# anihcsam/OpenGaussian

Measured on AMD Instinct MI355X. Metric: fwd+bwd Mpix/s at 1080p, 1M Gaussians (RGB+6-D ins_feat); k-means it/s, higher is better.
Workload: dtype f32; 1 GPU; S1M-1080p RGB(SH3)+depth+alpha (all grads) + 6-ch ins_feat (grad to ins_feat) fwd+bwd, ONE fused 9-channel pass; gaussians=1000000, width=1920, height=1080, views_cycled=8, parallelism=single

## Files before the change

include/ogs_raster.h:

```cpp
#ifndef OGS_RASTER_H
#define OGS_RASTER_H

#include <stddef.h>
#include <stdint.h>

#ifdef __cplusplus
extern "C" {
#endif

#define OGS_OK 0
#define OGS_ERR_INVALID_ARG (-1)
#define OGS_ERR_HIP (-2)
#define OGS_ERR_UNSUPPORTED (-3)
#define OGS_ERR_SCRATCH_TOO_SMALL (-4)
#define OGS_ERR_DEVICE (-5)

#define OGS_TILE 16
#define OGS_MAX_CHANNELS 12

typedef struct OgsRasterFwdArgs {
    int32_t P;
    int32_t W, H;
    int32_t C;
    int32_t sh_degree;
// ... 73 lines not shown
} OgsRasterBwdArgs;

int ogs_version(void);
const char* ogs_last_error(void);

int ogs_check_async_status(void);

size_t ogs_raster_geom_bytes(int32_t P, int32_t C);
size_t ogs_raster_geom_tmp_bytes(int32_t P);
size_t ogs_raster_image_bytes(int32_t W, int32_t H);
size_t ogs_raster_image_bytes_grouped(int32_t W, int32_t H, int32_t num_groups);
size_t ogs_raster_binning_tmp_bytes(int64_t num_rendered, int32_t W, int32_t H);
size_t ogs_raster_backward_tmp_bytes(int32_t P);
size_t ogs_raster_sorted_bytes(int64_t num_rendered, int32_t C);
size_t ogs_raster_quad_list_bytes(int64_t num_rendered);

int ogs_raster_forward_geometry(const OgsRasterFwdArgs* args, void* stream, int64_t* num_rendered_host);

int ogs_raster_forward_render(const OgsRasterFwdArgs* args, int64_t num_rendered, void* stream);

int ogs_raster_read_num_rendered_async(const OgsRasterFwdArgs* args, void* stream, uint32_t* host_pinned);
int ogs_raster_forward_render_deferred(const OgsRasterFwdArgs* args, int64_t capacity, void* stream);

int ogs_raster_read_num_emitted(const OgsRasterFwdArgs* args, void* stream, uint32_t* host);

size_t ogs_raster_tiny_max_points(void);
int ogs_raster_forward_tiny(const OgsRasterFwdArgs* args, void* stream);

size_t ogs_raster_tile_sort_capacity(int32_t level);

int ogs_raster_tile_count_debug(int64_t D, int64_t tiles, int32_t force_blocks, int32_t reverse);
size_t ogs_raster_tile_count_trip(void);

int ogs_raster_forward_reblend(const OgsRasterFwdArgs* args, void* stream);

int ogs_raster_compact_kept(int32_t W, int32_t H, int32_t C, const void* image_buffer, const void* sorted_rec,
                            const void* quad_list, void* new_image_buffer, void* new_sorted_rec, void* new_quad_list,
                            void* stream);

typedef struct OgsGroupStatsArgs {
    const int32_t* labels;
    int32_t num_labels;
    float alpha_threshold;
    float* max_alpha;
    int64_t* count;
    float* feat_sum;
    void* stats_tmp;
} OgsGroupStatsArgs;

size_t ogs_raster_stats_image_bytes(int32_t W, int32_t H, int32_t num_groups);
size_t ogs_raster_stats_tmp_bytes(int32_t num_groups, int32_t num_labels, int32_t C);
int ogs_raster_forward_group_stats(const OgsRasterFwdArgs* args, const OgsGroupStatsArgs* stats, int64_t num_rendered,
                                   void* stream);

int ogs_raster_backward(const OgsRasterBwdArgs* args, void* stream);

int ogs_mark_visible(int32_t P, const float* means3D, const float* viewmatrix, const float* projmatrix,
                     uint8_t* present, void* stream);

int ogs_sh_grad_from_views(int32_t P, int32_t V, int32_t sh_degree, int32_t sh_coeffs, const float* means3D,
                           const float* campos, const float* dL_drgb, float* dL_dsh, void* stream);

int ogs_raster_export_binning(const OgsRasterFwdArgs* args, int64_t num_rendered, uint64_t* keys_out,
                              uint32_t* ranges_out, uint32_t* n_contrib_out, void* stream);

int ogs_prof_enable(int on);
// ... 17 lines not shown
```

opengaussian_amd/_lib.py:

```python
from __future__ import annotations

import ctypes as C
import os

_HERE = os.path.dirname(os.path.abspath(__file__))
LIB_PATH = os.environ.get("OGS_LIB_PATH") or os.path.join(_HERE, "lib", "libogs_hip.so")

_f32p = C.POINTER(C.c_float)
_vp = C.c_void_p


class OgsRasterFwdArgs(C.Structure):
    _fields_ = [
        ("P", C.c_int32), ("W", C.c_int32), ("H", C.c_int32), ("C", C.c_int32),
        ("sh_degree", C.c_int32), ("sh_coeffs", C.c_int32),
        ("tanfovx", C.c_float), ("tanfovy", C.c_float), ("scale_modifier", C.c_float),
        ("prefiltered", C.c_int32), ("debug", C.c_int32),
        ("bg", _vp), ("means3D", _vp), ("colors_precomp", _vp), ("shs", _vp), ("opacities", _vp),
        ("scales", _vp), ("rotations", _vp), ("cov3D_precomp", _vp),
        ("viewmatrix", _vp), ("projmatrix", _vp), ("campos", _vp),
        ("out_color", _vp), ("out_depth", _vp), ("out_alpha", _vp), ("radii", _vp),
        ("geom_buffer", _vp), ("geom_tmp", _vp), ("image_buffer", _vp), ("point_list", _vp),
        ("binning_tmp", _vp), ("sorted_rec", _vp), ("quad_list", _vp), ("group_ids", _vp), ("num_groups", C.c_int32),
        ("full_binning", C.c_int32),
# ... 59 lines not shown

class OgsRawModel(C.Structure):
    _fields_ = [("features_dc", _vp), ("features_rest", _vp), ("scaling", _vp), ("rotation", _vp), ("opacity", _vp)]


class OgsRawModelGrads(C.Structure):
    _fields_ = [("features_dc", _vp), ("features_rest", _vp), ("scaling", _vp), ("rotation", _vp), ("opacity", _vp)]


SIGNATURES = {
    "ogs_version": (C.c_int, []),
    "ogs_last_error": (C.c_char_p, []),
    "ogs_raster_geom_bytes": (C.c_size_t, [C.c_int32, C.c_int32]),
    "ogs_raster_geom_tmp_bytes": (C.c_size_t, [C.c_int32]),
    "ogs_raster_image_bytes": (C.c_size_t, [C.c_int32, C.c_int32]),
    "ogs_raster_image_bytes_grouped": (C.c_size_t, [C.c_int32, C.c_int32, C.c_int32]),
    "ogs_raster_binning_tmp_bytes": (C.c_size_t, [C.c_int64, C.c_int32, C.c_int32]),
    "ogs_raster_backward_tmp_bytes": (C.c_size_t, [C.c_int32]),
    "ogs_raster_sorted_bytes": (C.c_size_t, [C.c_int64, C.c_int32]),
    "ogs_raster_quad_list_bytes": (C.c_size_t, [C.c_int64]),
    "ogs_raster_forward_geometry": (C.c_int, [C.POINTER(OgsRasterFwdArgs), _vp, C.POINTER(C.c_int64)]),
    "ogs_raster_forward_render": (C.c_int, [C.POINTER(OgsRasterFwdArgs), C.c_int64, _vp]),
    "ogs_raster_read_num_rendered_async": (C.c_int, [C.POINTER(OgsRasterFwdArgs), _vp, _vp]),
    "ogs_raster_forward_render_deferred": (C.c_int, [C.POINTER(OgsRasterFwdArgs), C.c_int64, _vp]),
    "ogs_raster_read_num_emitted": (C.c_int, [C.POINTER(OgsRasterFwdArgs), _vp, C.POINTER(C.c_uint32)]),
    "ogs_raster_stats_image_bytes": (C.c_size_t, [C.c_int32, C.c_int32, C.c_int32]),
    "ogs_raster_stats_tmp_bytes": (C.c_size_t, [C.c_int32, C.c_int32, C.c_int32]),
    "ogs_raster_forward_group_stats": (C.c_int, [C.POINTER(OgsRasterFwdArgs), C.POINTER(OgsGroupStatsArgs), C.c_int64, _vp]),
    "ogs_raster_backward": (C.c_int, [C.POINTER(OgsRasterBwdArgs), _vp]),
    "ogs_raster_tiny_max_points": (C.c_size_t, []),
    "ogs_raster_tile_sort_capacity": (C.c_size_t, [C.c_int32]),
    "ogs_raster_tile_count_debug": (C.c_int, [C.c_int64, C.c_int64, C.c_int32, C.c_int32]),
    "ogs_raster_tile_count_trip": (C.c_size_t, []),
    "ogs_raster_forward_tiny": (C.c_int, [C.POINTER(OgsRasterFwdArgs), _vp]),
    "ogs_raster_forward_reblend": (C.c_int, [C.POINTER(OgsRasterFwdArgs), _vp]),
    "ogs_raster_compact_kept": (C.c_int, [C.c_int32, C.c_int32, C.c_int32, _vp, _vp, _vp, _vp, _vp, _vp, _vp]),
    "ogs_mark_visible": (C.c_int, [C.c_int32, _vp, _vp, _vp, _vp, _vp]),
    "ogs_sh_grad_from_views": (C.c_int, [C.c_int32, C.c_int32, C.c_int32, C.c_int32, _vp, _vp, _vp, _vp, _vp]),
    "ogs_raster_export_binning": (C.c_int, [C.POINTER(OgsRasterFwdArgs), C.c_int64, _vp, _vp, _vp, _vp]),
    "ogs_selftest_wave_fold16": (C.c_int, [_vp, _vp, _vp]),
    "ogs_selftest_mfma_rank1": (C.c_int, [_vp, _vp, _vp, C.c_int32, _vp, _vp, _vp]),
    "ogs_selftest_tile_order": (C.c_int, [_vp, C.c_int64, _vp, _vp]),
    "ogs_selftest_radix_tmp_bytes": (C.c_size_t, [C.c_int64]),
    "ogs_selftest_radix_sort": (C.c_int, [_vp, _vp, _vp, _vp, C.c_int64, C.c_int32, C.c_int32, C.c_int32, _vp, _vp, _vp, _vp]),
    "ogs_raster_forward_geometry_raw": (C.c_int, [C.POINTER(OgsRasterFwdArgs), C.POINTER(OgsRawModel), _vp,
                                                  C.POINTER(C.c_int64)]),
    "ogs_raster_forward_tiny_raw": (C.c_int, [C.POINTER(OgsRasterFwdArgs), C.POINTER(OgsRawModel), _vp]),
    "ogs_raster_backward_raw": (C.c_int, [C.POINTER(OgsRasterBwdArgs), C.POINTER(OgsRawModel), C.POINTER(OgsRawModelGrads), _vp]),
    "ogs_model_activate": (C.c_int, [C.c_int32, C.c_int32, C.POINTER(OgsRawModel), _vp, _vp, _vp, _vp, _vp]),
    "ogs_check_async_status": (C.c_int, []),
    "ogs_prof_enable": (C.c_int, [C.c_int]),
    "ogs_prof_filter": (C.c_int, [C.c_char_p]),
    "ogs_prof_collect": (C.c_int, [C.c_char_p, C.c_size_t]),
    "ogs_kmeans_tmp_bytes": (C.c_size_t, [C.c_int64, C.c_int32, C.c_int32]),
    "ogs_kmeans_lloyd": (C.c_int, [_vp, C.c_int64, C.c_int32, _vp, C.c_int32, C.c_int32, C.c_int32, C.c_int32,
                                   _vp, C.c_int64, _vp, _vp]),
    "ogs_kmeans_assign": (C.c_int, [_vp, C.c_int64, C.c_int32, _vp, C.c_int32, _vp, C.c_int64, _vp]),
    "ogs_mask_feature_sums": (C.c_int, [_vp, _vp, _vp, C.c_int32, C.c_int32, C.c_int64, C.c_int32, _vp, _vp]),
    "ogs_mask_feature_sqdev": (C.c_int, [_vp, _vp, _vp, _vp, C.c_int32, C.c_int32, C.c_int64, _vp, _vp]),
    "ogs_mask_feature_sums_backward": (C.c_int, [_vp, _vp, _vp, _vp, _vp, C.c_int32, C.c_int32, C.c_int64, _vp, _vp, _vp]),
    "ogs_mask_cohesion": (C.c_int, [_vp, _vp, _vp, C.c_int32, C.c_int32, C.c_int64, _vp, _vp]),
    "ogs_mask_cohesion_backward": (C.c_int, [_vp, _vp, _vp, _vp, C.c_int32, C.c_int32, C.c_int64, _vp, _vp, _vp]),
    "ogs_label_feature_sums": (C.c_int, [_vp, _vp, _vp, C.c_int32, C.c_int32, C.c_int64, C.c_int32, _vp, _vp]),
    "ogs_label_feature_sqdev": (C.c_int, [_vp, _vp, _vp, _vp, C.c_int32, C.c_int32, C.c_int64, _vp, _vp]),
    "ogs_label_feature_sums_backward": (C.c_int, [_vp, _vp, _vp, _vp, _vp, C.c_int32, C.c_int32, C.c_int64, _vp, _vp, _vp]),
    "ogs_label_cohesion": (C.c_int, [_vp, _vp, _vp, C.c_int32, C.c_int32, C.c_int64, _vp, _vp]),
# ... 144 lines not shown
```

opengaussian_amd/csrc/binning.hip:

```cpp
#include <stdlib.h>
#include <string.h>

#include "ogs_common.h"

namespace ogs {

namespace {

constexpr size_t kSweepHeaderWords = 4 * 256 + 4 + 60;
constexpr int kScanItems = 8;
constexpr int kScanTile = kBlock * kScanItems;

__device__ __forceinline__ uint32_t wave_inclusive_scan(uint32_t v) {
#pragma unroll
    for (int d = 1; d < kWave; d <<= 1) {
        uint32_t t = __shfl_up(v, d, kWave);
        if (lane_id() >= d) v += t;
    }
    return v;
}

__device__ __forceinline__ uint32_t block_exclusive_scan(uint32_t v, uint32_t& total, uint32_t* wave_sums ) {
    const int wave = threadIdx.x >> 6;
    const uint32_t inc = wave_inclusive_scan(v);
    if (lane_id() == kWave - 1) wave_sums[wave] = inc;
    __syncthreads();
    uint32_t base = 0, tot = 0;
#pragma unroll
    for (int w = 0; w < kBlock / kWave; ++w) {
        const uint32_t s = wave_sums[w];
        if (w < wave) base += s;
        tot += s;
    }
    total = tot;
// ... 393 lines not shown
    const int64_t D = n_dev ? min((int64_t)*n_dev, D_cap) : D_cap;
    const int64_t i0 = ((int64_t)blockIdx.x * kBlock + threadIdx.x) * kRangeItems;
    if (i0 >= D) return;
    uint32_t k[kRangeItems];
    if (i0 + kRangeItems <= D) {
        const uint4 v = *reinterpret_cast<const uint4*>(tile_keys + i0);
        k[0] = v.x; k[1] = v.y; k[2] = v.z; k[3] = v.w;
    } else {
#pragma unroll
        for (int j = 0; j < kRangeItems; ++j) k[j] = i0 + j < D ? tile_keys[i0 + j] : 0u;
    }
    uint32_t prev = i0 > 0 ? tile_keys[i0 - 1] : 0u;
#pragma unroll
    for (int j = 0; j < kRangeItems; ++j) {
        const int64_t i = i0 + j;
        if (i < D) {
            const uint32_t cur = k[j];
            if (i == 0) {
                ranges[cur].x = 0;
            } else if (prev != cur) {
                ranges[prev].y = (uint32_t)i;
                ranges[cur].x = (uint32_t)i;
            }
            if (i == D - 1) ranges[cur].y = (uint32_t)D;
            prev = cur;
        }
    }
}

constexpr int kCountBlock = 1024;
constexpr int kCountItems = 4;
constexpr int kCountTrip = kCountBlock * kCountItems;
constexpr int kCountScanCols = 64, kCountScanGroups = 16;

__device__ __forceinline__ void tile_count_chunk(const uint32_t* __restrict__ n_dev, int64_t n_cap, int nchunks, int64_t& begin,
                                                 int64_t& end) {
    const int64_t n = n_dev ? min((int64_t)*n_dev, n_cap) : n_cap;
    const int64_t per = (n + nchunks - 1) / nchunks;
    const int64_t chunk = (per + kCountTrip - 1) / kCountTrip * kCountTrip;
    begin = min(n, (int64_t)blockIdx.x * chunk);
    end = min(n, begin + chunk);
}

__global__ __launch_bounds__(kCountBlock) void tile_count_kernel(const uint32_t* __restrict__ keys, int64_t n_cap,
                                                                 const uint32_t* __restrict__ n_dev, int tiles,
                                                                 uint32_t* __restrict__ table ) {
    extern __shared__ uint32_t count_lds[];
    int64_t begin, end;
    tile_count_chunk(n_dev, n_cap, (int)gridDim.x, begin, end);
    for (int t = threadIdx.x; t < tiles; t += kCountBlock) count_lds[t] = 0u;
    __syncthreads();
    for (int64_t i0 = begin + (int64_t)threadIdx.x * kCountItems; i0 < end; i0 += kCountTrip) {
        uint32_t k[kCountItems];
        if (i0 + kCountItems <= end) {
            const uint4 v = *reinterpret_cast<const uint4*>(keys + i0);
            k[0] = v.x; k[1] = v.y; k[2] = v.z; k[3] = v.w;
        } else {
#pragma unroll
            for (int j = 0; j < kCountItems; ++j) k[j] = i0 + j < end ? keys[i0 + j] : kDropKey;
        }
#pragma unroll
        for (int j = 0; j < kCountItems; ++j)
            if (k[j] < (uint32_t)tiles) atomicAdd(&count_lds[k[j]], 1u);
    }
    __syncthreads();
    uint32_t* row = table + (size_t)blockIdx.x * tiles;
    for (int t = threadIdx.x; t < tiles; t += kCountBlock) row[t] = count_lds[t];
}

__global__ __launch_bounds__(kCountScanCols * kCountScanGroups) void tile_count_scan_kernel(uint32_t* __restrict__ table, int nrows,
                                                                                            int tiles) {
    __shared__ uint32_t part[kCountScanGroups][kCountScanCols];
    const int c = threadIdx.x & (kCountScanCols - 1), g = threadIdx.x / kCountScanCols;
    const int t = blockIdx.x * kCountScanCols + c;
    const int per = (nrows + kCountScanGroups - 1) / kCountScanGroups;
    const int r0 = min(nrows, g * per), r1 = min(nrows, r0 + per);
    uint32_t sum = 0;
    if (t < tiles) {
#pragma unroll 8
        for (int r = r0; r < r1; ++r) sum += table[(size_t)r * tiles + t];
    }
    part[g][c] = sum;
    __syncthreads();
    uint32_t run = 0, total = 0;
#pragma unroll
    for (int j = 0; j < kCountScanGroups; ++j) {
        const uint32_t v = part[j][c];
        if (j < g) run += v;
        total += v;
    }
    if (t >= tiles) return;
    if (g == 0) table[(size_t)nrows * tiles + t] = total;
#pragma unroll 8
    for (int r = r0; r < r1; ++r) {
        uint32_t* p = table + (size_t)r * tiles + t;
        const uint32_t v = *p;
        *p = run;
        run += v;
    }
}

__global__ __launch_bounds__(kCountBlock) void tile_place_kernel(const uint32_t* __restrict__ keys, const uint32_t* __restrict__ vals,
                                                                 int64_t n_cap, const uint32_t* __restrict__ n_dev, int tiles,
                                                                 const uint32_t* __restrict__ table, uint2* __restrict__ ranges,
                                                                 uint32_t* __restrict__ kept, uint32_t* __restrict__ out,
                                                                 uint32_t out_cap, bool reverse) {
    extern __shared__ uint32_t count_lds[];
    __shared__ uint32_t wave_sums[kCountBlock / kWave];
    int64_t begin, end;
    tile_count_chunk(n_dev, n_cap, (int)gridDim.x, begin, end);
    if (begin >= end && blockIdx.x != 0) return;
    const uint32_t* totals = table + (size_t)gridDim.x * tiles;
    const uint32_t* row = table + (size_t)blockIdx.x * tiles;
    for (int t = threadIdx.x; t < tiles; t += kCountBlock) count_lds[t] = totals[t];
    __syncthreads();
    const int per = ((tiles + kCountBlock - 1) / kCountBlock) | 1;
    const int t0 = min(tiles, (int)threadIdx.x * per), t1 = min(tiles, t0 + per);
    uint32_t sum = 0;
    for (int t = t0; t < t1; ++t) sum += count_lds[t];
    const uint32_t inc = wave_inclusive_scan(sum);
    if (lane_id() == kWave - 1) wave_sums[threadIdx.x >> 6] = inc;
    __syncthreads();
    uint32_t run = inc - sum, total = 0;
#pragma unroll
    for (int w = 0; w < kCountBlock / kWave; ++w) {
        const uint32_t v = wave_sums[w];
        if (w < (int)(threadIdx.x >> 6)) run += v;
        total += v;
    }
    for (int t = t0; t < t1; ++t) {
        const uint32_t cnt = count_lds[t];
        count_lds[t] = run;
        run += cnt;
    }
    __syncthreads();
    if (blockIdx.x == 0) {
        for (int t = threadIdx.x; t < tiles; t += kCountBlock) {
            const uint32_t cnt = totals[t], start = count_lds[t];
            ranges[t] = cnt ? make_uint2(start, start + cnt) : make_uint2(0u, 0u);
        }
        if (threadIdx.x == 0) *kept = total;
    }
    for (int t = threadIdx.x; t < tiles; t += kCountBlock) count_lds[t] += row[t];
    __syncthreads();
    for (int64_t j0 = (int64_t)threadIdx.x * kCountItems; j0 < end - begin; j0 += kCountTrip) {
        uint32_t k[kCountItems], v[kCountItems];
        if (!reverse && begin + j0 + kCountItems <= end) {
            const uint4 kk = *reinterpret_cast<const uint4*>(keys + begin + j0);
            const uint4 vv = *reinterpret_cast<const uint4*>(vals + begin + j0);
            k[0] = kk.x; k[1] = kk.y; k[2] = kk.z; k[3] = kk.w;
            v[0] = vv.x; v[1] = vv.y; v[2] = vv.z; v[3] = vv.w;
        } else {
#pragma unroll
            for (int j = 0; j < kCountItems; ++j) {
                const int64_t i = reverse ? end - 1 - (j0 + j) : begin + j0 + j;
                const bool in = j0 + j < end - begin;
                k[j] = in ? keys[i] : kDropKey;
                v[j] = in ? vals[i] : 0u;
            }
        }
#pragma unroll
        for (int j = 0; j < kCountItems; ++j) {
            if (k[j] < (uint32_t)tiles) {
                const uint32_t pos = atomicAdd(&count_lds[k[j]], 1u);
                if (pos < out_cap) out[pos] = v[j];
            }
        }
    }
}

constexpr int kTileSortWaves = kBlock / kWave;
struct TileSortLds {
    uint32_t hist[kTileSortWaves][256];
    uint32_t dig_start[256];
    uint32_t base[256];
    uint32_t scan_sums[4];
    uint32_t red[2];
    uint2 range[kTileSortWaves];
    uint32_t kv[2 * kTileSortCap];
};
typedef __attribute__((address_space(3))) volatile uint32_t LdsWord;
typedef __attribute__((address_space(3))) unsigned long long LdsMask;
__device__ __forceinline__ LdsWord* lds_words(uint32_t* p) { return (LdsWord*)p; }
__device__ __forceinline__ LdsMask* wave_masks(TileSortLds& sm, int wave) { return (LdsMask*)(sm.kv + wave * 2 * kWaveSortCap); }

__device__ __forceinline__ void wave_rank_clear(LdsWord* hist, LdsMask* masks) {
    const int lane = threadIdx.x & (kWave - 1);
#pragma unroll
    for (int j = 0; j < 4; ++j) {
        hist[lane + j * kWave] = 0u;
        __hip_atomic_store(&masks[lane + j * kWave], 0ull, __ATOMIC_SEQ_CST, __HIP_MEMORY_SCOPE_WAVEFRONT);
    }
    __builtin_amdgcn_wave_barrier();
}

__device__ __forceinline__ void wave_rank(LdsWord* hist, LdsMask* masks, const uint32_t (&key)[kTileSortItems],
                                          uint32_t (&rank)[kTileSortItems], int ipl, int first, int m, int shift,
                                          uint32_t mask) {
    const int lane = threadIdx.x & (kWave - 1);
    const unsigned long long me = 1ull << lane;
// ... 558 lines not shown
        OGS_LAUNCH(radix_scatter_kernel<8>, dim3(nb), dim3(kBlock), 0, stream, keys_in, vals_in, keys_out, vals_out, n, n_dev,
                   shift, bits, (const uint32_t*)hist, (const uint32_t*)row_total, nb, drop, kept_out);
    }
    OGS_LAUNCH_CHECK(debug, stream);
    return OGS_OK;
}

int launch_tile_ranges(const uint32_t* tile_keys_sorted, int64_t D, uint2* ranges, int64_t tiles, hipStream_t s,
                       int debug, const uint32_t* n_dev, bool already_zeroed) {
    if (!already_zeroed) OGS_HIP_CHECK(hipMemsetAsync(ranges, 0, (size_t)tiles * sizeof(uint2), s));
    if (D <= 0) return OGS_OK;
    const int grid = (int)((D + (int64_t)kBlock * kRangeItems - 1) / ((int64_t)kBlock * kRangeItems));
    OGS_LAUNCH(tile_ranges_kernel, dim3(grid), dim3(kBlock), 0, s, tile_keys_sorted, D, n_dev, ranges);
    OGS_LAUNCH_CHECK(debug, s);
    return OGS_OK;
}

static int g_tile_count_force = 0;
static bool g_tile_place_reverse = false;
void tile_count_debug(int force_blocks, int reverse) {
    if (force_blocks >= 0) g_tile_count_force = force_blocks;
    if (reverse >= 0) g_tile_place_reverse = reverse != 0;
}
int tile_count_trip() { return kCountTrip; }

int tile_count_blocks(int64_t D, int64_t tiles) {
    if (tiles < 1 || tiles > kTileCountMaxTiles || D < 2 * tiles) return 0;
    const int64_t trips = (D + kCountTrip - 1) / kCountTrip;
    int64_t B = g_tile_count_force > 0 ? g_tile_count_force : (trips < kTileCountBlocks ? trips : kTileCountBlocks);
    if (B > D / tiles - 1) B = D / tiles - 1;
    return (int)B;
}

int launch_tile_count_binning(const uint32_t* keys, const uint32_t* vals, int64_t D, const uint32_t* n_dev, int B, int64_t tiles,
                              uint32_t* table, uint2* ranges, uint32_t* kept, uint32_t* point_list, hipStream_t s, int debug) {
    if (B < 1 || tiles < 1 || tiles > kTileCountMaxTiles || ((int64_t)B + 1) * tiles > D) {
        set_error("tile_count_binning: B=%d tiles=%lld D=%lld", B, (long long)tiles, (long long)D); return OGS_ERR_INVALID_ARG;
    }
    const size_t lds = (size_t)tiles * sizeof(uint32_t);
    OGS_LAUNCH(tile_count_kernel, dim3(B), dim3(kCountBlock), lds, s, keys, D, n_dev, (int)tiles, table);
    OGS_LAUNCH_CHECK(debug, s);
    const int cols = (int)((tiles + kCountScanCols - 1) / kCountScanCols);
    OGS_LAUNCH(tile_count_scan_kernel, dim3(cols), dim3(kCountScanCols * kCountScanGroups), 0, s, table, B, (int)tiles);
    OGS_LAUNCH_CHECK(debug, s);
    OGS_LAUNCH(tile_place_kernel, dim3(B), dim3(kCountBlock), lds, s, keys, vals, D, n_dev, (int)tiles, (const uint32_t*)table,
               ranges, kept, point_list, (uint32_t)D, g_tile_place_reverse);
    OGS_LAUNCH_CHECK(debug, s);
    return OGS_OK;
}

int launch_tile_depth_sort(const uint2* ranges, int64_t tiles, const uint32_t* tile_order, uint32_t* point_list,
                           const uint32_t* depth_keys, uint32_t* scratch, hipStream_t s, int debug) {
    if (tiles <= 0) return OGS_OK;
    if (tiles >= (1ll << 31)) { set_error("tile_depth_sort: %lld tiles", (long long)tiles); return OGS_ERR_UNSUPPORTED; }
    const unsigned grid = (unsigned)((tiles + kTileSortWaves - 1) / kTileSortWaves);
    OGS_LAUNCH(tile_depth_sort_kernel, dim3(grid), dim3(kBlock), 0, s, ranges, (int)tiles, tile_order, point_list, depth_keys,
               scratch);
    OGS_LAUNCH_CHECK(debug, s);
    return OGS_OK;
}

int launch_export_keys(const uint2* ranges, int tiles, const uint32_t* point_list, const float4* rec, int recv4,
                       uint64_t* keys_out, hipStream_t s) {
    OGS_LAUNCH(export_keys_kernel, dim3(tiles), dim3(kBlock), 0, s, ranges, point_list, rec, recv4, keys_out);
    OGS_LAUNCH_CHECK(0, s);
    return OGS_OK;
}

}
```

opengaussian_amd/csrc/capi.hip:

```cpp
#include <stdarg.h>
#include <stdlib.h>
#include <string.h>

#include <map>
#include <mutex>
#include <string>
#include <vector>

#include "ogs_common.h"

namespace ogs {

static thread_local char g_err[512] = "";

void set_error(const char* fmt, ...) {
    va_list ap;
    va_start(ap, fmt);
    vsnprintf(g_err, sizeof(g_err), fmt, ap);
    va_end(ap);
}

namespace {
struct ProfRec { const char* name; hipEvent_t start, stop; };
int g_prof_mode = 0;
// ... 424 lines not shown
        set_error("forward_reblend: NULL required pointer (colors_precomp, bg, out_*, image_buffer, sorted_rec, quad_list)");
        return OGS_ERR_INVALID_ARG;
    }
    const int rc = check_async_status("forward_reblend (entry)");
    if (rc != OGS_OK) return rc;
    const ImageState is = ImageState::carve(a->image_buffer, a->W, a->H, 1);
    return launch_reblend(*a, is, static_cast<hipStream_t>(stream_));
}

int ogs_raster_compact_kept(int32_t W, int32_t H, int32_t C, const void* image_buffer, const void* sorted_rec, const void* quad_list,
                            void* new_image_buffer, void* new_sorted_rec, void* new_quad_list, void* stream_) {
    if (W <= 0 || H <= 0) { set_error("compact_kept: bad sizes W=%d H=%d", W, H); return OGS_ERR_INVALID_ARG; }
    if (!image_buffer || !sorted_rec || !quad_list || !new_image_buffer || !new_sorted_rec || !new_quad_list) {
        set_error("compact_kept: NULL pointer"); return OGS_ERR_INVALID_ARG;
    }
    const ImageState is_old = ImageState::carve(const_cast<void*>(image_buffer), W, H, 1);
    const ImageState is_new = ImageState::carve(new_image_buffer, W, H, 1);
    return launch_compact_kept(W, H, C, is_old, is_new, sorted_rec, quad_list, new_sorted_rec, new_quad_list,
                               static_cast<hipStream_t>(stream_));
}

size_t ogs_raster_tiny_max_points(void) { return (size_t)kTinyMaxP; }

size_t ogs_raster_tile_sort_capacity(int32_t level) {
    return level == 0 ? (size_t)kWaveSortCap : level == 1 ? (size_t)kTileSortCap : 0;
}

int ogs_raster_tile_count_debug(int64_t D, int64_t tiles, int32_t force_blocks, int32_t reverse) {
    tile_count_debug(force_blocks, reverse);
    return tile_count_blocks(D, tiles);
}
size_t ogs_raster_tile_count_trip(void) { return (size_t)tile_count_trip(); }

static int forward_tiny_impl(const OgsRasterFwdArgs* a_in, void* stream_, bool raw, const float* raw_rest) {
    int rc = validate_fwd(a_in);
    if (rc != OGS_OK) return rc;
    OgsRasterFwdArgs a_raw;
    const OgsRasterFwdArgs* a = a_in;
    if (raw) { a_raw = *a_in; a_raw.cov3D_precomp = raw_rest; a = &a_raw; }
    if (a->P <= 0 || a->P > kTinyMaxP) { set_error("forward_tiny: P=%d outside [1, %d]", a->P, kTinyMaxP); return OGS_ERR_INVALID_ARG; }
    if (a->num_groups > 1) { set_error("forward_tiny: grouped passes use the streaming path"); return OGS_ERR_UNSUPPORTED; }
    hipStream_t s = static_cast<hipStream_t>(stream_);
    const GeomState gs = GeomState::carve(a->geom_buffer, a->P, a->C);
    uint32_t* order = static_cast<uint32_t*>(a->geom_tmp);
    rc = launch_tiny_geometry(*a, gs, order, s, raw);
    if (rc != OGS_OK) return rc;
    return launch_tiny_blend(*a, gs, order, s);
}

int ogs_raster_forward_tiny(const OgsRasterFwdArgs* a, void* stream_) { return forward_tiny_impl(a, stream_, false, nullptr); }

int ogs_raster_forward_tiny_raw(const OgsRasterFwdArgs* a, const OgsRawModel* raw, void* stream_) {
    OgsRasterFwdArgs b;
    const int rc = raw_fwd_args(a, raw, &b);
    if (rc != OGS_OK) return rc;
    return forward_tiny_impl(&b, stream_, true, raw->features_rest);
}

static int backward_impl(const OgsRasterBwdArgs* a, void* stream_, const OgsRawModelGrads* raw_grads) {
    if (!a) { set_error("args == NULL"); return OGS_ERR_INVALID_ARG; }
    if (a->C != 3 && a->C != 6 && a->C != 9) { set_error("backward: C=%d unsupported (3, 6, 9)", a->C); return OGS_ERR_UNSUPPORTED; }
    if (a->P == 0) return OGS_OK;
    const bool feat_only = backward_is_features_only(*a);
    if (!a->dL_dcolor || !a->image_buffer || !a->bwd_tmp || !a->radii) {
        set_error("backward: NULL required pointer"); return OGS_ERR_INVALID_ARG;
    }
// ... 164 lines not shown
```

opengaussian_amd/csrc/ogs_common.h:

```cpp
#pragma once

#include <hip/hip_runtime.h>
#include <stdint.h>
#include <stddef.h>
#include <stdio.h>
#include <type_traits>

#include "../../include/ogs_raster.h"
#include "../../include/ogs_model.h"

namespace ogs {

constexpr int kTile = OGS_TILE;
constexpr int kBlock = 256;
constexpr int kWave = 64;
constexpr int kTinyMaxP = 256;
constexpr int kSmallMaxP = 1024;

void set_error(const char* fmt, ...);

#define OGS_HIP_CHECK(expr)                                                              \
    do {                                                                                 \
        hipError_t _e = (expr);                                                          \
        if (_e != hipSuccess) {                                                          \
// ... 242 lines not shown
        b.kept = c.take<uint32_t>(1);
        b.sort_tmp = c.take<char>(sort_tmp_bytes(D));
        return b;
    }
    static size_t bytes(int64_t D) {
        Carver c(nullptr);
        for (int i = 0; i < 3; ++i) c.take<uint32_t>(D);
        c.take<uint32_t>(1);
        c.take<char>(sort_tmp_bytes(D));
        return c.off;
    }
};

int launch_preprocess(const OgsRasterFwdArgs& a, const GeomState& gs, const GeomTmp& gt, hipStream_t s, bool raw = false);
int launch_block_offsets(const OgsRasterFwdArgs& a, const GeomTmp& gt, hipStream_t s);
int launch_tiny_geometry(const OgsRasterFwdArgs& a, const GeomState& gs, uint32_t* order, hipStream_t s, bool raw = false);
int launch_small_geometry(const OgsRasterFwdArgs& a, const GeomState& gs, const GeomTmp& gt, hipStream_t s, bool raw = false);
int launch_model_activate(int P, int M, const OgsRawModel& raw, float* scales, float* rotations, float* opacities, float* shs,
                          hipStream_t s);
int launch_tiny_blend(const OgsRasterFwdArgs& a, const GeomState& gs, const uint32_t* order, hipStream_t s);
int launch_reblend(const OgsRasterFwdArgs& a, const ImageState& is, hipStream_t s);
int launch_compact_kept(int W, int H, int C, const ImageState& is_old, const ImageState& is_new, const void* old_rec,
                        const void* old_quad, void* new_rec, void* new_quad, hipStream_t s);
int launch_duplicate(const OgsRasterFwdArgs& a, const GeomState& gs, const GeomTmp& gt, uint32_t* tile_keys,
                     uint32_t* vals, uint32_t capacity, bool drop_unreachable, bool depth_order, hipStream_t s,
                     uint2* zero_ranges = nullptr, int n_zero = 0);
int launch_tile_ranges(const uint32_t* tile_keys_sorted, int64_t D, uint2* ranges, int64_t tiles, hipStream_t s,
                       int debug, const uint32_t* n_dev = nullptr, bool already_zeroed = false);
constexpr int kTileCountMaxTiles = 12288;
constexpr int kTileCountBlocks = 128;
int tile_count_blocks(int64_t D, int64_t tiles);
int tile_count_trip();
void tile_count_debug(int force_blocks, int reverse);
int launch_tile_count_binning(const uint32_t* keys, const uint32_t* vals, int64_t D, const uint32_t* n_dev, int B, int64_t tiles,
                              uint32_t* table, uint2* ranges, uint32_t* kept, uint32_t* point_list, hipStream_t s, int debug);
inline bool per_tile_depth_order(const OgsRasterFwdArgs& a) { return a.num_groups <= 1 && a.P > kSmallMaxP; }
inline bool block_sum_offsets(const OgsRasterFwdArgs& a) { return per_tile_depth_order(a) && a.full_binning == 0; }
constexpr int kTileSortItems = 16;
constexpr int kTileSortCap = kBlock * kTileSortItems;
constexpr int kWaveSortCap = kTileSortCap / (kBlock / kWave);
int launch_tile_depth_sort(const uint2* ranges, int64_t tiles, const uint32_t* tile_order, uint32_t* point_list,
                           const uint32_t* depth_keys, uint32_t* scratch, hipStream_t s, int debug);
inline int num_groups_of(int g) { return g > 1 ? g : 1; }
int launch_group_stats(const OgsRasterFwdArgs& a, const OgsGroupStatsArgs& st, const GeomState& gs, const ImageState& is,
                       hipStream_t s, bool order_ready = false);
int launch_blend_forward(const OgsRasterFwdArgs& a, const GeomState& gs, const ImageState& is, int64_t D,
                         hipStream_t s, bool order_ready = false);
int launch_blend_backward(const OgsRasterBwdArgs& a, const ImageState& is, void* grad_rec, hipStream_t s);
int launch_preprocess_backward(const OgsRasterBwdArgs& a, const GeomState& gs, const void* grad_rec, hipStream_t s,
                               const OgsRawModelGrads* raw_grads = nullptr);
inline bool backward_is_features_only(const OgsRasterBwdArgs& a) {
    return a.dL_dcolors != nullptr && a.colors_precomp != nullptr && !a.dL_dmeans2D && !a.dL_dopacity &&
           !a.dL_dmeans3D && !a.dL_dcov3D && !a.dL_dsh && !a.dL_dscales && !a.dL_drotations && !a.dL_dsh_rgb;
}
int launch_sh_grad_from_views(int P, int V, int sh_degree, int sh_coeffs, const float* means3D, const float* campos,
                              const float* dL_drgb, float* dL_dsh, hipStream_t s);
int launch_wave_fold16_test(const float* in, float* out, hipStream_t s);
int launch_mfma_rank1_test(const float* w, const float* f, const float* acc0, int steps, float* out_mfma, float* out_fma,
                           hipStream_t s);
int launch_tile_order_test(const uint32_t* ranges, int64_t vtiles, uint32_t* order, hipStream_t s);
int launch_mark_visible(int P, const float* means3D, const float* viewmatrix, uint8_t* present, hipStream_t s);
int launch_export_keys(const uint2* ranges, int tiles, const uint32_t* point_list, const float4* rec, int recv4,
                       uint64_t* keys_out, hipStream_t s);

__device__ __forceinline__ float blend_power(float a2, float b2, float c2, float dx, float dy) {
    const float u = fmaf(b2, dy, a2 * dx);
// ... 52 lines not shown
```

Baseline: 1544 Mpix/s.

## Split tile placement across tile slices and stage scattered writes in LDS

The tile placement kernel now launches a 2-D grid: chunks of the sorted key stream by slices of the tile range, so each block only keeps offsets for its own slice of tiles in LDS. That raises the number of blocks in flight. When the block's entries fit, they are first staged in LDS with their tile index and then written to the point list in contiguous runs, replacing random global scatter with coalesced stores. The cost is that each slice re-reads the whole key chunk and does extra prefix sums, and the kernel needs a larger dynamic LDS allocation that must be raised via a function attribute. Debug hooks expose and override the plan.

After: 1563 Mpix/s, median of 6. 1.01x the previous value.

```diff
diff --git a/include/ogs_raster.h b/include/ogs_raster.h
--- a/include/ogs_raster.h
+++ b/include/ogs_raster.h
@@ -129,6 +129,8 @@
 int ogs_raster_tile_count_debug(int64_t D, int64_t tiles, int32_t force_blocks, int32_t reverse);
 size_t ogs_raster_tile_count_trip(void);
 
+int ogs_raster_tile_place_debug(int64_t D, int64_t tiles, int32_t group, int32_t slices, int32_t stage_words, int32_t* chosen);
+
 int ogs_raster_forward_reblend(const OgsRasterFwdArgs* args, void* stream);
 
 int ogs_raster_compact_kept(int32_t W, int32_t H, int32_t C, const void* image_buffer, const void* sorted_rec,
diff --git a/opengaussian_amd/_lib.py b/opengaussian_amd/_lib.py
--- a/opengaussian_amd/_lib.py
+++ b/opengaussian_amd/_lib.py
@@ -115,6 +115,7 @@
     "ogs_raster_tile_sort_capacity": (C.c_size_t, [C.c_int32]),
     "ogs_raster_tile_count_debug": (C.c_int, [C.c_int64, C.c_int64, C.c_int32, C.c_int32]),
     "ogs_raster_tile_count_trip": (C.c_size_t, []),
+    "ogs_raster_tile_place_debug": (C.c_int, [C.c_int64, C.c_int64, C.c_int32, C.c_int32, C.c_int32, C.POINTER(C.c_int32)]),
     "ogs_raster_forward_tiny": (C.c_int, [C.POINTER(OgsRasterFwdArgs), _vp]),
     "ogs_raster_forward_reblend": (C.c_int, [C.POINTER(OgsRasterFwdArgs), _vp]),
     "ogs_raster_compact_kept": (C.c_int, [C.c_int32, C.c_int32, C.c_int32, _vp, _vp, _vp, _vp, _vp, _vp, _vp]),
diff --git a/opengaussian_amd/csrc/binning.hip b/opengaussian_amd/csrc/binning.hip
--- a/opengaussian_amd/csrc/binning.hip
+++ b/opengaussian_amd/csrc/binning.hip
@@ -1,5 +1,7 @@
 #include <stdlib.h>
 #include <string.h>
+
+#include <atomic>
 
 #include "ogs_common.h"
 
@@ -459,14 +461,21 @@
 constexpr int kCountItems = 4;
 constexpr int kCountTrip = kCountBlock * kCountItems;
 constexpr int kCountScanCols = 64, kCountScanGroups = 16;
-
-__device__ __forceinline__ void tile_count_chunk(const uint32_t* __restrict__ n_dev, int64_t n_cap, int nchunks, int64_t& begin,
-                                                 int64_t& end) {
+constexpr int kPlaceUnroll = 2;
+constexpr int kPlaceEntryBytes = 6;
+
+__device__ __forceinline__ void tile_chunk_span(const uint32_t* __restrict__ n_dev, int64_t n_cap, int nchunks, int p, int group,
+                                                int64_t& begin, int64_t& end) {
     const int64_t n = n_dev ? min((int64_t)*n_dev, n_cap) : n_cap;
     const int64_t per = (n + nchunks - 1) / nchunks;
     const int64_t chunk = (per + kCountTrip - 1) / kCountTrip * kCountTrip;
-    begin = min(n, (int64_t)blockIdx.x * chunk);
-    end = min(n, begin + chunk);
+    begin = min(n, (int64_t)p * group * chunk);
+    end = min(n, begin + (int64_t)group * chunk);
+}
+
+__device__ __forceinline__ void tile_count_chunk(const uint32_t* __restrict__ n_dev, int64_t n_cap, int nchunks, int64_t& begin,
+                                                 int64_t& end) {
+    tile_chunk_span(n_dev, n_cap, nchunks, (int)blockIdx.x, 1, begin, end);
 }
 
 __global__ __launch_bounds__(kCountBlock) void tile_count_kernel(const uint32_t* __restrict__ keys, int64_t n_cap,
@@ -527,72 +536,132 @@
     }
 }
 
+template <bool kStaged>
+__device__ __forceinline__ void tile_place_walk(const uint32_t* __restrict__ keys, const uint32_t* __restrict__ vals, int64_t begin,
+                                                int64_t end, bool reverse, uint32_t ulo, uint32_t unt, uint32_t* cur,
+                                                uint32_t* stage, uint16_t* stile, uint32_t stage_words, uint32_t* __restrict__ out,
+                                                uint32_t out_cap) {
+    const int64_t len = end - begin;
+    for (int64_t i0 = (int64_t)threadIdx.x * kCountItems; i0 < len; i0 += (int64_t)kPlaceUnroll * kCountTrip) {
+        uint32_t k[kPlaceUnroll][kCountItems], v[kPlaceUnroll][kCountItems];
+#pragma unroll
+        for (int u = 0; u < kPlaceUnroll; ++u) {
+            const int64_t iu = i0 + (int64_t)u * kCountTrip;
+            if (!reverse && begin + iu + kCountItems <= end) {
+                const uint4 kk = *reinterpret_cast<const uint4*>(keys + begin + iu);
+                const uint4 vv = *reinterpret_cast<const uint4*>(vals + begin + iu);
+                k[u][0] = kk.x - ulo; k[u][1] = kk.y - ulo; k[u][2] = kk.z - ulo; k[u][3] = kk.w - ulo;
+                v[u][0] = vv.x; v[u][1] = vv.y; v[u][2] = vv.z; v[u][3] = vv.w;
+            } else {
+#pragma unroll
+                for (int j = 0; j < kCountItems; ++j) {
+                    const int64_t i = reverse ? end - 1 - (iu + j) : begin + iu + j;
+                    const bool in = iu + j < len;
+                    k[u][j] = in ? keys[i] - ulo : kDropKey;
+                    v[u][j] = in ? vals[i] : 0u;
+                }
+            }
+        }
+#pragma unroll
+        for (int u = 0; u < kPlaceUnroll; ++u) {
+#pragma unroll
+            for (int j = 0; j < kCountItems; ++j) {
+                if (k[u][j] < unt) {
+                    const uint32_t pos = atomicAdd(&cur[k[u][j]], 1u);
+                    if (kStaged) {
+                        if (pos < stage_words) {
+                            stage[pos] = v[u][j];
+                            stile[pos] = (uint16_t)k[u][j];
+                        }
+                    } else if (pos < out_cap) {
+                        out[pos] = v[u][j];
+                    }
+                }
+            }
+        }
+    }
+}
+
 __global__ __launch_bounds__(kCountBlock) void tile_place_kernel(const uint32_t* __restrict__ keys, const uint32_t* __restrict__ vals,
                                                                  int64_t n_cap, const uint32_t* __restrict__ n_dev, int tiles,
+                                                                 int nrows, int group, uint32_t stage_words,
                                                                  const uint32_t* __restrict__ table, uint2* __restrict__ ranges,
                                                                  uint32_t* __restrict__ kept, uint32_t* __restrict__ out,
                                                                  uint32_t out_cap, bool reverse) {
     extern __shared__ uint32_t count_lds[];
-    __shared__ uint32_t wave_sums[kCountBlock / kWave];
+    __shared__ uint32_t wave_sums[3][kCountBlock / kWave];
+    const int p = blockIdx.x, slices = gridDim.y;
+    const int per_slice = (tiles + slices - 1) / slices;
+    const int t_lo = min(tiles, (int)blockIdx.y * per_slice), nt = min(tiles, t_lo + per_slice) - t_lo;
     int64_t begin, end;
-    tile_count_chunk(n_dev, n_cap, (int)gridDim.x, begin, end);
-    if (begin >= end && blockIdx.x != 0) return;
-    const uint32_t* totals = table + (size_t)gridDim.x * tiles;
-    const uint32_t* row = table + (size_t)blockIdx.x * tiles;
-    for (int t = threadIdx.x; t < tiles; t += kCountBlock) count_lds[t] = totals[t];
-    __syncthreads();
-    const int per = ((tiles + kCountBlock - 1) / kCountBlock) | 1;
-    const int t0 = min(tiles, (int)threadIdx.x * per), t1 = min(tiles, t0 + per);
-    uint32_t sum = 0;
-    for (int t = t0; t < t1; ++t) sum += count_lds[t];
-    const uint32_t inc = wave_inclusive_scan(sum);
-    if (lane_id() == kWave - 1) wave_sums[threadIdx.x >> 6] = inc;
-    __syncthreads();
-    uint32_t run = inc - sum, total = 0;
+    tile_chunk_span(n_dev, n_cap, nrows, p, group, begin, end);
+    if (begin >= end && p != 0) return;
+    const bool may_stage = stage_words > 0;
+    uint32_t* cur = count_lds;
+    uint32_t* delta = cur + per_slice;
+    uint32_t* stage = delta + per_slice;
+    const uint32_t* totals = table + (size_t)nrows * tiles;
+    const uint32_t* row = table + (size_t)p * group * tiles + t_lo;
+    const uint32_t* row_end = table + (size_t)min(nrows, (p + 1) * group) * tiles + t_lo;
+    uint32_t front = 0;
+    for (int t = threadIdx.x; t < t_lo; t += kCountBlock) front += totals[t];
+    for (int j = threadIdx.x; j < nt; j += kCountBlock) {
+        cur[j] = totals[t_lo + j];
+        if (may_stage) delta[j] = row_end[j] - row[j];
+    }
+    __syncthreads();
+    const int per = ((nt + kCountBlock - 1) / kCountBlock) | 1;
+    const int j0 = min(nt, (int)threadIdx.x * per), j1 = min(nt, j0 + per);
+    uint32_t sum = 0, mine = 0;
+    for (int j = j0; j < j1; ++j) {
+        sum += cur[j];
+        if (may_stage) mine += delta[j];
+    }
+    const uint32_t inc = wave_inclusive_scan(sum), inc_mine = wave_inclusive_scan(mine), inc_front = wave_inclusive_scan(front);
+    if (lane_id() == kWave - 1) {
+        wave_sums[0][threadIdx.x >> 6] = inc;
+        wave_sums[1][threadIdx.x >> 6] = inc_mine;
+        wave_sums[2][threadIdx.x >> 6] = inc_front;
+    }
+    __syncthreads();
+    uint32_t run = inc - sum, run_mine = inc_mine - mine, total = 0, need = 0;
 #pragma unroll
     for (int w = 0; w < kCountBlock / kWave; ++w) {
-        const uint32_t v = wave_sums[w];
-        if (w < (int)(threadIdx.x >> 6)) run += v;
-        total += v;
-    }
-    for (int t = t0; t < t1; ++t) {
-        const uint32_t cnt = count_lds[t];
-        count_lds[t] = run;
+        const uint32_t a = wave_sums[0][w], b = wave_sums[1][w];
+        if (w < (int)(threadIdx.x >> 6)) { run += a; run_mine += b; }
+        total += a + wave_sums[2][w];
+        run += wave_sums[2][w];
+        need += b;
+    }
+    const bool staged = may_stage && need <= stage_words;
+    for (int j = j0; j < j1; ++j) {
+        const uint32_t cnt = cur[j], c = may_stage ? delta[j] : 0u;
+        if (p == 0) ranges[t_lo + j] = cnt ? make_uint2(run, run + cnt) : make_uint2(0u, 0u);
+        if (staged) {
+            cur[j] = run_mine;
+            delta[j] = run - run_mine;
+        } else {
+            cur[j] = run;
+        }
         run += cnt;
-    }
-    __syncthreads();
-    if (blockIdx.x == 0) {
-        for (int t = threadIdx.x; t < tiles; t += kCountBlock) {
-            const uint32_t cnt = totals[t], start = count_lds[t];
-            ranges[t] = cnt ? make_uint2(start, start + cnt) : make_uint2(0u, 0u);
-        }
-        if (threadIdx.x == 0) *kept = total;
-    }
-    for (int t = threadIdx.x; t < tiles; t += kCountBlock) count_lds[t] += row[t];
-    __syncthreads();
-    for (int64_t j0 = (int64_t)threadIdx.x * kCountItems; j0 < end - begin; j0 += kCountTrip) {
-        uint32_t k[kCountItems], v[kCountItems];
-        if (!reverse && begin + j0 + kCountItems <= end) {
-            const uint4 kk = *reinterpret_cast<const uint4*>(keys + begin + j0);
-            const uint4 vv = *reinterpret_cast<const uint4*>(vals + begin + j0);
-            k[0] = kk.x; k[1] = kk.y; k[2] = kk.z; k[3] = kk.w;
-            v[0] = vv.x; v[1] = vv.y; v[2] = vv.z; v[3] = vv.w;
-        } else {
-#pragma unroll
-            for (int j = 0; j < kCountItems; ++j) {
-                const int64_t i = reverse ? end - 1 - (j0 + j) : begin + j0 + j;
-                const bool in = j0 + j < end - begin;
-                k[j] = in ? keys[i] : kDropKey;
-                v[j] = in ? vals[i] : 0u;
-            }
-        }
-#pragma unroll
-        for (int j = 0; j < kCountItems; ++j) {
-            if (k[j] < (uint32_t)tiles) {
-                const uint32_t pos = atomicAdd(&count_lds[k[j]], 1u);
-                if (pos < out_cap) out[pos] = v[j];
-            }
-        }
+        run_mine += c;
+    }
+    if (p == 0 && blockIdx.y == gridDim.y - 1 && threadIdx.x == 0) *kept = total;
+    if (begin >= end || nt == 0 || (may_stage && need == 0)) return;
+    __syncthreads();
+    for (int j = threadIdx.x; j < nt; j += kCountBlock) (staged ? delta : cur)[j] += row[j];
+    __syncthreads();
+    const uint32_t ulo = (uint32_t)t_lo, unt = (uint32_t)nt;
+    uint16_t* stile = reinterpret_cast<uint16_t*>(stage + stage_words);
+    if (!staged) {
+        tile_place_walk<false>(keys, vals, begin, end, reverse, ulo, unt, cur, stage, stile, stage_words, out, out_cap);
+        return;
+    }
+    tile_place_walk<true>(keys, vals, begin, end, reverse, ulo, unt, cur, stage, stile, stage_words, out, out_cap);
+    __syncthreads();
+    for (uint32_t i = threadIdx.x; i < need; i += kCountBlock) {
+        const uint32_t pos = delta[min((int)stile[i], nt - 1)] + i;
+        if (pos < out_cap) out[pos] = stage[i];
     }
 }
 
@@ -1217,6 +1286,39 @@
     return (int)B;
 }
 
+static int g_tile_place_group = 0, g_tile_place_slices = 0, g_tile_place_stage = 0;
+void tile_place_debug(int group, int slices, int stage_words) {
+    if (group >= 0) g_tile_place_group = group;
+    if (slices >= 0) g_tile_place_slices = slices;
+    if (stage_words >= 0) g_tile_place_stage = stage_words;
+}
+
+constexpr size_t kPlaceLdsBytes = 160 * 1024 - 256;
+constexpr int kPlaceMaxSlices = 1024;
+constexpr int kPlaceGrid = 256, kPlaceOwnSlices = 4;
+constexpr int kPlaceStageTrips = 2;
+
+TilePlacePlan tile_place_plan(int64_t D, int64_t tiles, int B) {
+    TilePlacePlan pl = {0, 0, 0, 0};
+    if (B < 1 || tiles < 1) return pl;
+    const bool rule = D >= (int64_t)kPlaceStageTrips * kCountTrip * B;
+    int G = 1, S = 1;
+    if (rule) S = kPlaceGrid / B < 1 ? 1 : kPlaceGrid / B > kPlaceOwnSlices ? kPlaceOwnSlices : kPlaceGrid / B;
+    if (g_tile_place_group > 0) G = g_tile_place_group;
+    if (g_tile_place_slices > 0) S = g_tile_place_slices < kPlaceMaxSlices ? g_tile_place_slices : kPlaceMaxSlices;
+    if (G > B) G = B;
+    const int64_t per_slice = (tiles + S - 1) / S;
+    const int64_t room = ((int64_t)kPlaceLdsBytes - 8 * per_slice) / kPlaceEntryBytes;
+    const int64_t span = G * (((D + B - 1) / B + kCountTrip - 1) / kCountTrip * kCountTrip);
+    int64_t W = g_tile_place_stage > 0 ? g_tile_place_stage : (rule || G > 1 || S > 1) ? span : 0;
+    if (W > room) W = room;
+    pl.group = G;
+    pl.chunks = (B + G - 1) / G;
+    pl.slices = S;
+    pl.stage_words = (uint32_t)W;
+    return pl;
+}
+
 int launch_tile_count_binning(const uint32_t* keys, const uint32_t* vals, int64_t D, const uint32_t* n_dev, int B, int64_t tiles,
                               uint32_t* table, uint2* ranges, uint32_t* kept, uint32_t* point_list, hipStream_t s, int debug) {
     if (B < 1 || tiles < 1 || tiles > kTileCountMaxTiles || ((int64_t)B + 1) * tiles > D) {
@@ -1228,8 +1330,22 @@
     const int cols = (int)((tiles + kCountScanCols - 1) / kCountScanCols);
     OGS_LAUNCH(tile_count_scan_kernel, dim3(cols), dim3(kCountScanCols * kCountScanGroups), 0, s, table, B, (int)tiles);
     OGS_LAUNCH_CHECK(debug, s);
-    OGS_LAUNCH(tile_place_kernel, dim3(B), dim3(kCountBlock), lds, s, keys, vals, D, n_dev, (int)tiles, (const uint32_t*)table,
-               ranges, kept, point_list, (uint32_t)D, g_tile_place_reverse);
+    const TilePlacePlan pl = tile_place_plan(D, tiles, B);
+    const size_t per_slice = (size_t)((tiles + pl.slices - 1) / pl.slices);
+    const size_t place_lds = pl.stage_words ? (8 * per_slice + (size_t)kPlaceEntryBytes * pl.stage_words + 15) / 16 * 16
+                                            : per_slice * sizeof(uint32_t);
+    if (place_lds > 48 * 1024) {
+        static std::atomic<bool> raised[64];
+        int dev = 0;
+        OGS_HIP_CHECK(hipGetDevice(&dev));
+        if (dev < 0 || dev >= 64 || !raised[dev].load(std::memory_order_relaxed)) {
+            OGS_HIP_CHECK(hipFuncSetAttribute(reinterpret_cast<const void*>(tile_place_kernel),
+                                              hipFuncAttributeMaxDynamicSharedMemorySize, (int)kPlaceLdsBytes));
+            if (dev >= 0 && dev < 64) raised[dev].store(true, std::memory_order_relaxed);
+        }
+    }
+    OGS_LAUNCH(tile_place_kernel, dim3(pl.chunks, pl.slices), dim3(kCountBlock), place_lds, s, keys, vals, D, n_dev, (int)tiles, B,
+               pl.group, pl.stage_words, (const uint32_t*)table, ranges, kept, point_list, (uint32_t)D, g_tile_place_reverse);
     OGS_LAUNCH_CHECK(debug, s);
     return OGS_OK;
 }
diff --git a/opengaussian_amd/csrc/capi.hip b/opengaussian_amd/csrc/capi.hip
--- a/opengaussian_amd/csrc/capi.hip
+++ b/opengaussian_amd/csrc/capi.hip
@@ -480,6 +480,15 @@
 }
 size_t ogs_raster_tile_count_trip(void) { return (size_t)tile_count_trip(); }
 
+int ogs_raster_tile_place_debug(int64_t D, int64_t tiles, int32_t group, int32_t slices, int32_t stage_words, int32_t* chosen) {
+    tile_place_debug(group, slices, stage_words);
+    if (chosen) {
+        const TilePlacePlan pl = tile_place_plan(D, tiles, tile_count_blocks(D, tiles));
+        chosen[0] = pl.chunks; chosen[1] = pl.slices; chosen[2] = (int32_t)pl.stage_words;
+    }
+    return OGS_OK;
+}
+
 static int forward_tiny_impl(const OgsRasterFwdArgs* a_in, void* stream_, bool raw, const float* raw_rest) {
     int rc = validate_fwd(a_in);
     if (rc != OGS_OK) return rc;
diff --git a/opengaussian_amd/csrc/ogs_common.h b/opengaussian_amd/csrc/ogs_common.h
--- a/opengaussian_amd/csrc/ogs_common.h
+++ b/opengaussian_amd/csrc/ogs_common.h
@@ -298,6 +298,9 @@
 int tile_count_blocks(int64_t D, int64_t tiles);
 int tile_count_trip();
 void tile_count_debug(int force_blocks, int reverse);
+struct TilePlacePlan { int group, chunks, slices; uint32_t stage_words; };
+TilePlacePlan tile_place_plan(int64_t D, int64_t tiles, int B);
+void tile_place_debug(int group, int slices, int stage_words);
 int launch_tile_count_binning(const uint32_t* keys, const uint32_t* vals, int64_t D, const uint32_t* n_dev, int B, int64_t tiles,
                               uint32_t* table, uint2* ranges, uint32_t* kept, uint32_t* point_list, hipStream_t s, int debug);
 inline bool per_tile_depth_order(const OgsRasterFwdArgs& a) { return a.num_groups <= 1 && a.P > kSmallMaxP; }
```
